# facebookresearch/PartDistillation

Hardware: AMD Instinct MI355X
Metric: images/sec training step, R50 Mask2Former 1024² bs=2/GPU, 1/2/4/8 MI355X (higher is better)
Workload: dtype bf16

## Files before the change

### partdistillation_amd/csrc/attention.hip

```cpp
#include <hip/hip_runtime.h>
#include <math.h>
#include <stdint.h>

#include "pd_attention.h"
#include "pd_common.h"
#include "mfma_bf16.h"
#include "pd_msda.h"

int g_attn_bwd_kc = 0;

namespace {

constexpr int D = 32;
constexpr int QP = 128;
constexpr int KT = 64;
constexpr int KC_FWD = 256;
constexpr int KC_DQ = 512;

typedef unsigned short bf16_t;

__device__ __forceinline__ float bf2f(bf16_t h) { return __uint_as_float((unsigned)h << 16); }
__device__ __forceinline__ bf16_t f2bf(float f)
{
  unsigned u = __float_as_uint(f);
  if ((u & 0x7fffffffu) > 0x7f800000u) return (bf16_t)((u >> 16) | 0x40);
  u += 0x7fffu + ((u >> 16) & 1u);
  return (bf16_t)(u >> 16);
}

template <typename T> struct IO;
template <> struct IO<float> {
  static __device__ __forceinline__ void load32(const float *p, float *dst)
  {
#pragma unroll
    for (int i = 0; i < 8; ++i) {
      const float4 v = reinterpret_cast<const float4 *>(p)[i];
      dst[4 * i] = v.x; dst[4 * i + 1] = v.y; dst[4 * i + 2] = v.z; dst[4 * i + 3] = v.w;
    }
  }
  static __device__ __forceinline__ void store32(float *p, const float *src)
  {
#pragma unroll
    for (int i = 0; i < 8; ++i) reinterpret_cast<float4 *>(p)[i] = make_float4(src[4 * i], src[4 * i + 1], src[4 * i + 2], src[4 * i + 3]);
  }
  static __device__ __forceinline__ void load8(const float *p, float *dst)
  {
    const float4 a = reinterpret_cast<const float4 *>(p)[0], b = reinterpret_cast<const float4 *>(p)[1];
    dst[0] = a.x; dst[1] = a.y; dst[2] = a.z; dst[3] = a.w; dst[4] = b.x; dst[5] = b.y; dst[6] = b.z; dst[7] = b.w;
  }
};
template <> struct IO<bf16_t> {
  static __device__ __forceinline__ void load8(const bf16_t *p, float *dst)
  {
    const uint4 v = *reinterpret_cast<const uint4 *>(p);
    const unsigned w[4] = {v.x, v.y, v.z, v.w};
#pragma unroll
    for (int i = 0; i < 4; ++i) { dst[2 * i] = __uint_as_float(w[i] << 16); dst[2 * i + 1] = __uint_as_float(w[i] & 0xffff0000u); }
  }
  static __device__ __forceinline__ void load32(const bf16_t *p, float *dst)
  {
#pragma unroll
    for (int i = 0; i < 4; ++i) load8(p + 8 * i, dst + 8 * i);
  }
  static __device__ __forceinline__ void store32(bf16_t *p, const float *src)
  {
#pragma unroll
    for (int i = 0; i < 4; ++i) {
      uint4 v;
      unsigned *w = &v.x;
#pragma unroll
      for (int j = 0; j < 4; ++j) w[j] = (unsigned)f2bf(src[8 * i + 2 * j]) | ((unsigned)f2bf(src[8 * i + 2 * j + 1]) << 16);
      reinterpret_cast<uint4 *>(p)[i] = v;
    }
  }
};

template <typename T>
__device__ __forceinline__ void stage_rows(const T *__restrict__ src, float (*dst)[D], int k0, int Lk, int b, int h, int B, int H)
{
  const int r = threadIdx.x >> 2, c = (threadIdx.x & 3) * 8;
  float tmp[8];
  if (k0 + r < Lk) IO<T>::load8(src + ((int64_t)(k0 + r) * B + b) * (H * D) + h * D + c, tmp);
  else {
#pragma unroll
    for (int i = 0; i < 8; ++i) tmp[i] = 0.f;
  }
#pragma unroll
  for (int i = 0; i < 8; ++i) dst[r][c + i] = tmp[i];
}

template <typename T>
__global__ __launch_bounds__(256) void attn_fwd_partial(const T *__restrict__ q, const T *__restrict__ k, const T *__restrict__ v,
// ... 200 lines not shown

template <typename T>
__global__ __launch_bounds__(256) void attn_bwd_dkv(const T *__restrict__ q, const T *__restrict__ k, const T *__restrict__ v,
                                                     const uint8_t *__restrict__ mask, const T *__restrict__ o, const T *__restrict__ d_o,
                                                     const float *__restrict__ lse, T *__restrict__ dk, T *__restrict__ dv, int B,
                                                     int H, int Lq, int Lk, float scale)
{
  __shared__ __attribute__((aligned(16))) float Qs[QS][D];
  __shared__ __attribute__((aligned(16))) float Os[QS][D];
  __shared__ float Ls[QS], Ds[QS];
  const int h = blockIdx.y, b = blockIdx.z;
  const int ki = blockIdx.x * 256 + threadIdx.x;
  const bool active = ki < Lk;
  float kv[D], vv[D], dkv[D], dvv[D];
#pragma unroll
  for (int d = 0; d < D; ++d) { dkv[d] = 0.f; dvv[d] = 0.f; }
  if (active) {
    const int64_t off = ((int64_t)ki * B + b) * (H * D) + h * D;
    IO<T>::load32(k + off, kv);
    IO<T>::load32(v + off, vv);
  }
  for (int q0 = 0; q0 < Lq; q0 += QS) {
    __syncthreads();
    {
      const int r = threadIdx.x >> 3, c = (threadIdx.x & 7) * 4;
      float part = 0.f;
      if (q0 + r < Lq) {
        const int64_t off = ((int64_t)(q0 + r) * B + b) * (H * D) + h * D + c;
#pragma unroll
        for (int i = 0; i < 4; ++i) {
          float qx, dox, ox;
          if (sizeof(T) == 2) {
            qx = bf2f(reinterpret_cast<const bf16_t *>(q)[off + i]); dox = bf2f(reinterpret_cast<const bf16_t *>(d_o)[off + i]);
            ox = bf2f(reinterpret_cast<const bf16_t *>(o)[off + i]);
          } else {
            qx = reinterpret_cast<const float *>(q)[off + i]; dox = reinterpret_cast<const float *>(d_o)[off + i];
            ox = reinterpret_cast<const float *>(o)[off + i];
          }
          Qs[r][c + i] = qx * scale; Os[r][c + i] = dox;
          part += dox * ox;
        }
      } else {
#pragma unroll
        for (int i = 0; i < 4; ++i) { Qs[r][c + i] = 0.f; Os[r][c + i] = 0.f; }
      }
      part += __shfl_xor(part, 1, 64); part += __shfl_xor(part, 2, 64); part += __shfl_xor(part, 4, 64);
      if ((threadIdx.x & 7) == 0) {
        Ds[r] = part;
        Ls[r] = (q0 + r < Lq) ? lse[((int64_t)b * H + h) * Lq + q0 + r] : -INFINITY;
      }
    }
    __syncthreads();
    if (!active) continue;
    const int nq = min(QS, Lq - q0);
    for (int r = 0; r < nq; ++r) {
      const float lq = Ls[r];
      if (lq == -INFINITY) continue;
      if (mask && mask[((int64_t)b * Lq + q0 + r) * Lk + ki]) continue;
      float s = 0.f, dp = 0.f;
#pragma unroll
      for (int d = 0; d < D; ++d) { s += Qs[r][d] * kv[d]; dp += Os[r][d] * vv[d]; }
      const float p = __expf(s - lq), ds = p * (dp - Ds[r]);
#pragma unroll
      for (int d = 0; d < D; ++d) { dkv[d] += ds * Qs[r][d]; dvv[d] += p * Os[r][d]; }
    }
  }
  if (active) {
    const int64_t off = ((int64_t)ki * B + b) * (H * D) + h * D;
    IO<T>::store32(dk + off, dkv);
    IO<T>::store32(dv + off, dvv);
  }
}

using pdmfma::bf16x4;
using pdmfma::f32x16;
using pdmfma::gather4;
using pdmfma::lds4;
using pdmfma::mma;
using pdmfma::pack4;

constexpr int LR = 36;
constexpr int LT = 132;
constexpr int MQ = 128;

__device__ __forceinline__ unsigned mask4(const uint8_t *row, int key0, int Lk, bool aligned)
{
  if (key0 >= Lk) return 0u;
  if (aligned) return *reinterpret_cast<const unsigned *>(row + key0);
  unsigned m = 0;
  for (int i = 0; i < 4; ++i)
    if (key0 + i < Lk) m |= (unsigned)row[key0 + i] << (8 * i);
  return m;
}

template <bool MASK>
__global__ __launch_bounds__(256) void attn_fwd_mfma(const bf16_t *__restrict__ q, const bf16_t *__restrict__ k,
                                                     const bf16_t *__restrict__ v, const uint8_t *__restrict__ mask,
                                                     bf16_t *__restrict__ o, float *__restrict__ lse, float *__restrict__ part_o,
                                                     float *__restrict__ part_ml, int B, int H, int Lq, int Lk, float scale,
                                                     int nchunk, int ldkv, int kc)
{
  __shared__ __attribute__((aligned(16))) bf16_t Ks[2][32][LR];
  __shared__ __attribute__((aligned(16))) bf16_t Vs[2][32][LR];
  const int chunk = blockIdx.x, h = blockIdx.y, b = blockIdx.z;
  const int tid = threadIdx.x, wave = tid >> 6, lane = tid & 63, r = lane & 31, hh = lane >> 5;
  const int qi = wave * 32 + r;
  const bool qvalid = qi < Lq;
  const int64_t rs = (int64_t)H * D;
  bf16x4 qreg[4];
#pragma unroll
  for (int s = 0; s < 4; ++s) {
    qreg[s] = bf16x4{0, 0, 0, 0};
    if (qvalid) qreg[s] = *reinterpret_cast<const bf16x4 *>(q + ((int64_t)qi * B + b) * rs + h * D + 8 * s + 4 * hh);
  }
  const int kbeg = chunk * kc, kend = min(Lk, kbeg + kc);
  const int ntile = (kend - kbeg + 31) / 32;
  const bf16_t *src = (tid < 128) ? k : v;
  const int srow = (tid & 127) >> 2, spiece = tid & 3;
  auto gload = [&](int t) {
    const int key = kbeg + 32 * t + srow;
    uint4 val = make_uint4(0, 0, 0, 0);
    if (key < kend) val = *reinterpret_cast<const uint4 *>(src + ((int64_t)key * B + b) * ldkv + h * D + spiece * 8);
    return val;
  };
  auto lstore = [&](int buf, uint4 val) {
    bf16_t *dst = ((tid < 128) ? &Ks[buf][srow][0] : &Vs[buf][srow][0]) + spiece * 8;
    *reinterpret_cast<uint2 *>(dst) = make_uint2(val.x, val.y);
    *reinterpret_cast<uint2 *>(dst + 4) = make_uint2(val.z, val.w);
  };
  const bool aligned = (Lk & 3) == 0;
  const uint8_t *mrow = (MASK && qvalid) ? mask + ((int64_t)b * Lq + qi) * Lk : nullptr;
  float m_run = -INFINITY, l_part = 0.f;
  f32x16 oacc;
#pragma unroll
  for (int e = 0; e < 16; ++e) oacc[e] = 0.f;
  if (ntile > 0) lstore(0, gload(0));
  __syncthreads();
  for (int t = 0; t < ntile; ++t) {
    const int buf = t & 1, kbase = kbeg + 32 * t;
    uint4 nxt = make_uint4(0, 0, 0, 0);
    if (t + 1 < ntile) nxt = gload(t + 1);
    f32x16 sacc;
#pragma unroll
    for (int e = 0; e < 16; ++e) sacc[e] = 0.f;
#pragma unroll
    for (int s = 0; s < 4; ++s) mma(sacc, lds4(&Ks[buf][r][8 * s + 4 * hh]), qreg[s]);
    float m_t = -INFINITY;
#pragma unroll
    for (int g = 0; g < 4; ++g) {
      const int key0 = kbase + 8 * g + 4 * hh;
      const unsigned m4 = mrow ? mask4(mrow, key0, Lk, aligned) : 0u;
#pragma unroll
      for (int i = 0; i < 4; ++i) {
        const bool blocked = (key0 + i >= kend) || ((m4 >> (8 * i)) & 0xffu);
        const float sv = blocked ? -INFINITY : sacc[4 * g + i] * scale;
        sacc[4 * g + i] = sv;
        m_t = fmaxf(m_t, sv);
      }
    }
    m_t = fmaxf(m_t, __shfl_xor(m_t, 32, 64));
    const float m_new = fmaxf(m_run, m_t);
    const bool dead = m_new == -INFINITY;
    const float alpha = dead ? 1.f : __expf(m_run - m_new);
    float psum = 0.f;
    bf16x4 preg[4];
#pragma unroll
// ... 149 lines not shown
#pragma unroll
          for (int s = 0; s < 4; ++s) { mma(sT, kreg[s], qreg[s]); mma(dpT, vreg[s], greg[s]); }
          const float lse_q = Ls[ql], delta_q = Ds[ql];
          unsigned mybits = 0;
          bf16x4 dsT[4];
#pragma unroll
          for (int g = 0; g < 4; ++g) {
            const int key0 = kbase + 8 * g + 4 * hh;
            const unsigned m4 = m4s[sub][g];
            float ds[4];
#pragma unroll
            for (int i = 0; i < 4; ++i) {
              const bool blocked = (key0 + i >= kend) || ((m4 >> (8 * i)) & 0xffu);
              const float p = blocked ? 0.f : __expf(sT[4 * g + i] * scale - lse_q);
              ds[i] = p * (dpT[4 * g + i] - delta_q);
              const unsigned long long bal = __ballot(blocked);
              if (r == 8 * g + i) mybits = (unsigned)bal;
              if (r == 8 * g + 4 + i) mybits = (unsigned)(bal >> 32);
            }
            dsT[g] = pack4(ds[0], ds[1], ds[2], ds[3]);
          }
#pragma unroll
          for (int j = 0; j < 4; ++j) mma(dqacc[sub], ktreg[j], dsT[j]);
          f32x16 sN, dpN;
#pragma unroll
          for (int e = 0; e < 16; ++e) { sN[e] = 0.f; dpN[e] = 0.f; }
#pragma unroll
          for (int s = 0; s < 4; ++s) { mma(sN, qreg[s], kreg[s]); mma(dpN, greg[s], vreg[s]); }
          bf16x4 pN[4], dsN[4];
#pragma unroll
          for (int g = 0; g < 4; ++g) {
            const float4 l4 = *reinterpret_cast<const float4 *>(&Ls[32 * sub + 8 * g + 4 * hh]);
            const float4 d4 = *reinterpret_cast<const float4 *>(&Ds[32 * sub + 8 * g + 4 * hh]);
            const float la[4] = {l4.x, l4.y, l4.z, l4.w}, da[4] = {d4.x, d4.y, d4.z, d4.w};
            float p[4], ds[4];
#pragma unroll
            for (int i = 0; i < 4; ++i) {
              const bool blocked = (mybits >> (8 * g + 4 * hh + i)) & 1u;
              p[i] = blocked ? 0.f : __expf(sN[4 * g + i] * scale - la[i]);
              ds[i] = p[i] * (dpN[4 * g + i] - da[i]);
            }
            pN[g] = pack4(p[0], p[1], p[2], p[3]);
            dsN[g] = pack4(ds[0], ds[1], ds[2], ds[3]);
          }
#pragma unroll
          for (int j = 0; j < 4; ++j) {
            mma(dvacc, lds4(&Ot[r][32 * sub + 8 * j + 4 * hh]), pN[j]);
            mma(dkacc, lds4(&Qt[r][32 * sub + 8 * j + 4 * hh]), dsN[j]);
          }
        }
      }
      if (kvalid) {
        bf16_t *dkp = dk + ((int64_t)key * B + b) * rs + h * D, *dvp = dv + ((int64_t)key * B + b) * rs + h * D;
#pragma unroll
        for (int g = 0; g < 4; ++g) {
          *reinterpret_cast<bf16x4 *>(dkp + 8 * g + 4 * hh) = pack4(dkacc[4 * g] * scale, dkacc[4 * g + 1] * scale, dkacc[4 * g + 2] * scale, dkacc[4 * g + 3] * scale);
          *reinterpret_cast<bf16x4 *>(dvp + 8 * g + 4 * hh) = pack4(dvacc[4 * g], dvacc[4 * g + 1], dvacc[4 * g + 2], dvacc[4 * g + 3]);
        }
      }
    }
  }
  for (int w = 0; w < 4; ++w) {
    __syncthreads();
    if (wave == w) {
#pragma unroll
      for (int sub = 0; sub < 4; ++sub)
#pragma unroll
        for (int e = 0; e < 16; ++e) {
          const int d = (e & 3) + 8 * (e >> 2) + 4 * hh;
          if (w == 0) dqs[32 * sub + r][d] = dqacc[sub][e];
          else dqs[32 * sub + r][d] += dqacc[sub][e];
        }
    }
  }
  __syncthreads();
  for (int idx = tid; idx < Lq * D; idx += 256) {
    const int qq = idx >> 5, d = idx & 31;
    const float val = dqs[qq][d] * scale;
    if (nchunk == 1) dq[((int64_t)qq * B + b) * rs + h * D + d] = f2bf(val);
    else part_dq[((bh * nchunk + chunk) * Lq + qq) * D + d] = val;
  }
}

inline int nchunks(int Lk, int kc) { return Lk <= 0 ? 1 : (Lk + kc - 1) / kc; }
inline int mfma_fwd_chunk(int B, int H, int Lk)
{
  int kc = KC_FWD;
  if (Lk > KC_FWD)
    while (kc > 64 && (int64_t)B * H * nchunks(Lk, kc) < 512) kc >>= 1;
  return kc;
}
inline int mfma_bwd_chunk(int B, int H, int Lk)
{
  if (g_attn_bwd_kc == 128 || g_attn_bwd_kc == 256 || g_attn_bwd_kc == 512) return g_attn_bwd_kc;
  int kc = KC_DQ;
  while (kc > 128 && (int64_t)B * H * nchunks(Lk, kc) < 256) kc >>= 1;
  return kc;
}

int check(const void *a, const void *b, const void *c, int B, int H, int Lq, int Lk, int dtype, const char *who)
{
  if (B < 0 || H <= 0 || Lq < 0 || Lk < 0) return pd_set_error(PD_ERR_INVALID_ARG, "%s: bad sizes B=%d H=%d Lq=%d Lk=%d", who, B, H, Lq, Lk);
  if (dtype != PD_F32 && dtype != PD_BF16) return pd_set_error(PD_ERR_INVALID_ARG, "%s: dtype %d (float32 / bfloat16 only)", who, dtype);
  if (B * Lq * Lk != 0 && (!a || !b || !c)) return pd_set_error(PD_ERR_INVALID_ARG, "%s: null pointer", who);
  return PD_OK;
}

}

int g_pd_dbg_attn_scalar = 0;

extern "C" int64_t pd_attn_workspace_floats(int B, int H, int Lq, int Lk)
{
  const int64_t n1 = (int64_t)B * H * nchunks(Lk, mfma_fwd_chunk(B, H, Lk)) * Lq * (D + 2);
  const int64_t n2 = (int64_t)B * H * nchunks(Lk, 128) * Lq * D;
  return (n1 > n2 ? n1 : n2) + 64;
}

extern "C" int pd_attn_fwd_d32(const void *q, const void *k, const void *v, const uint8_t *mask, void *o, float *lse,
                               float *workspace, int B, int H, int Lq, int Lk, float scale, int dtype, void *stream_)
{
  return pd_attn_fwd_d32_ld(q, k, v, mask, o, lse, workspace, B, H, Lq, Lk, scale, dtype, H * D, stream_);
}

extern "C" int pd_attn_fwd_d32_ld(const void *q, const void *k, const void *v, const uint8_t *mask, void *o, float *lse,
                                  float *workspace, int B, int H, int Lq, int Lk, float scale, int dtype, int ld_kv, void *stream_)
{
  int rc = check(q, k, v, B, H, Lq, Lk, dtype, "pd_attn_fwd_d32");
  if (rc) return rc;
  if (ld_kv < H * D || (ld_kv & 7)) return pd_set_error(PD_ERR_INVALID_ARG, "pd_attn_fwd_d32_ld: ld_kv=%d (>= H * 32, a multiple of 8)", ld_kv);
  if (ld_kv != H * D && !(dtype == PD_BF16 && Lq <= MQ && Lk > 0 && !g_pd_dbg_attn_scalar))
    return pd_set_error(PD_ERR_INVALID_ARG, "pd_attn_fwd_d32_ld: strided k / v only on the matrix-core path (bf16, <= %d queries)", MQ);
  if (B * Lq == 0) return PD_OK;
  if (!o || !lse || !workspace) return pd_set_error(PD_ERR_INVALID_ARG, "pd_attn_fwd_d32: null output");
  hipStream_t s = (hipStream_t)stream_;
  if (dtype == PD_BF16 && Lq <= MQ && Lk > 0 && !g_pd_dbg_attn_scalar) {
    const int kc = mfma_fwd_chunk(B, H, Lk), nc = nchunks(Lk, kc);
    float *part_o = workspace, *part_ml = workspace + (int64_t)B * H * nc * Lq * D;
    if (mask) hipLaunchKernelGGL(attn_fwd_mfma<true>, dim3(nc, H, B), dim3(256), 0, s, (const bf16_t *)q, (const bf16_t *)k, (const bf16_t *)v,
                                 mask, (bf16_t *)o, lse, part_o, part_ml, B, H, Lq, Lk, scale, nc, ld_kv, kc);
    else hipLaunchKernelGGL(attn_fwd_mfma<false>, dim3(nc, H, B), dim3(256), 0, s, (const bf16_t *)q, (const bf16_t *)k, (const bf16_t *)v,
                            mask, (bf16_t *)o, lse, part_o, part_ml, B, H, Lq, Lk, scale, nc, ld_kv, kc);
    if (nc > 1) hipLaunchKernelGGL(attn_fwd_combine<bf16_t>, dim3((B * H * Lq + 7) / 8), dim3(256), 0, s, part_o, part_ml, (bf16_t *)o, lse, B, H, Lq, nc);
    return pd_check_launch("pd_attn_fwd_d32");
  }
  const int nc = nchunks(Lk, KC_FWD);
  float *part_o = workspace, *part_ml = workspace + (int64_t)B * H * nc * Lq * D;
  for (int qp = 0; qp * QP < Lq; ++qp) {
    if (dtype == PD_BF16)
      hipLaunchKernelGGL(attn_fwd_partial<bf16_t>, dim3(nc, H, B), dim3(256), 0, s, (const bf16_t *)q, (const bf16_t *)k,
                         (const bf16_t *)v, mask, part_o, part_ml, B, H, Lq, Lk, scale, nc, qp);
    else
      hipLaunchKernelGGL(attn_fwd_partial<float>, dim3(nc, H, B), dim3(256), 0, s, (const float *)q, (const float *)k,
                         (const float *)v, mask, part_o, part_ml, B, H, Lq, Lk, scale, nc, qp);
  }
  const int groups = B * H * Lq;
  if (dtype == PD_BF16)
    hipLaunchKernelGGL(attn_fwd_combine<bf16_t>, dim3((groups + 7) / 8), dim3(256), 0, s, part_o, part_ml, (bf16_t *)o, lse, B, H, Lq, nc);
  else
    hipLaunchKernelGGL(attn_fwd_combine<float>, dim3((groups + 7) / 8), dim3(256), 0, s, part_o, part_ml, (float *)o, lse, B, H, Lq, nc);
  return pd_check_launch("pd_attn_fwd_d32");
}

extern "C" int pd_attn_bwd_d32(const void *q, const void *k, const void *v, const uint8_t *mask, const void *o, const void *d_o,
                               const float *lse, void *dq, void *dk, void *dv, float *workspace, int B, int H, int Lq,
                               int Lk, float scale, int dtype, void *stream_)
{
  return pd_attn_bwd_d32_ld(q, k, v, mask, o, d_o, lse, dq, dk, dv, workspace, B, H, Lq, Lk, scale, dtype, H * D, stream_);
}

extern "C" int pd_attn_bwd_d32_ld(const void *q, const void *k, const void *v, const uint8_t *mask, const void *o, const void *d_o,
                                  const float *lse, void *dq, void *dk, void *dv, float *workspace, int B, int H, int Lq,
                                  int Lk, float scale, int dtype, int ld_kv, void *stream_)
{
  int rc = check(q, k, v, B, H, Lq, Lk, dtype, "pd_attn_bwd_d32");
  if (rc) return rc;
  if (ld_kv < H * D || (ld_kv & 3)) return pd_set_error(PD_ERR_INVALID_ARG, "pd_attn_bwd_d32_ld: ld_kv=%d (>= H * 32, a multiple of 4)", ld_kv);
  if (ld_kv != H * D && !(dtype == PD_BF16 && Lq <= MQ && !g_pd_dbg_attn_scalar))
    return pd_set_error(PD_ERR_INVALID_ARG, "pd_attn_bwd_d32_ld: strided k / v only on the matrix-core path (bf16, <= %d queries)", MQ);
  hipStream_t s = (hipStream_t)stream_;
  if (B * Lq == 0) {
    const size_t bytes = (size_t)B * Lk * H * D * (dtype == PD_BF16 ? 2 : 4);
    if (bytes == 0) return PD_OK;
    if (!dk || !dv) return pd_set_error(PD_ERR_INVALID_ARG, "pd_attn_bwd_d32: null pointer");
    if (hipMemsetAsync(dk, 0, bytes, s) != hipSuccess || hipMemsetAsync(dv, 0, bytes, s) != hipSuccess)
      return pd_set_error(PD_ERR_LAUNCH, "pd_attn_bwd_d32: clearing dk / dv failed");
    return PD_OK;
  }
  const int groups = B * H * Lq;
  if (Lk == 0) {
    if (!dq) return pd_set_error(PD_ERR_INVALID_ARG, "pd_attn_bwd_d32: null pointer");
    if (dtype == PD_BF16) hipLaunchKernelGGL(attn_bwd_dq_reduce<bf16_t>, dim3((groups + 7) / 8), dim3(256), 0, s, workspace, (bf16_t *)dq, B, H, Lq, 0);
    else hipLaunchKernelGGL(attn_bwd_dq_reduce<float>, dim3((groups + 7) / 8), dim3(256), 0, s, workspace, (float *)dq, B, H, Lq, 0);
    return pd_check_launch("pd_attn_bwd_d32");
  }
  if (!o || !d_o || !lse || !dq || !dk || !dv || !workspace) return pd_set_error(PD_ERR_INVALID_ARG, "pd_attn_bwd_d32: null pointer");
  if (dtype == PD_BF16 && Lq <= MQ && !g_pd_dbg_attn_scalar) {
    const int kc = mfma_bwd_chunk(B, H, Lk), nc = nchunks(Lk, kc);
    if (mask) hipLaunchKernelGGL(attn_bwd_mfma<true>, dim3(nc, H, B), dim3(256), 0, s, (const bf16_t *)q, (const bf16_t *)k, (const bf16_t *)v,
                                 mask, (const bf16_t *)o, (const bf16_t *)d_o, lse, workspace, (bf16_t *)dq, (bf16_t *)dk, (bf16_t *)dv,
                                 B, H, Lq, Lk, scale, nc, kc, ld_kv);
    else hipLaunchKernelGGL(attn_bwd_mfma<false>, dim3(nc, H, B), dim3(256), 0, s, (const bf16_t *)q, (const bf16_t *)k, (const bf16_t *)v,
                            mask, (const bf16_t *)o, (const bf16_t *)d_o, lse, workspace, (bf16_t *)dq, (bf16_t *)dk, (bf16_t *)dv,
                            B, H, Lq, Lk, scale, nc, kc, ld_kv);
    if (nc > 1) hipLaunchKernelGGL(attn_bwd_dq_reduce<bf16_t>, dim3((groups + 7) / 8), dim3(256), 0, s, workspace, (bf16_t *)dq, B, H, Lq, nc);
    return pd_check_launch("pd_attn_bwd_d32");
  }
  const int nc = nchunks(Lk, KC_DQ);
  if (dtype == PD_BF16) {
    for (int qp = 0; qp * QP < Lq; ++qp)
      hipLaunchKernelGGL(attn_bwd_dq<bf16_t>, dim3(nc, H, B), dim3(256), 0, s, (const bf16_t *)q, (const bf16_t *)k, (const bf16_t *)v,
                         mask, (const bf16_t *)o, (const bf16_t *)d_o, lse, workspace, B, H, Lq, Lk, scale, nc, qp);
    hipLaunchKernelGGL(attn_bwd_dq_reduce<bf16_t>, dim3((groups + 7) / 8), dim3(256), 0, s, workspace, (bf16_t *)dq, B, H, Lq, nc);
    hipLaunchKernelGGL(attn_bwd_dkv<bf16_t>, dim3((Lk + 255) / 256, H, B), dim3(256), 0, s, (const bf16_t *)q, (const bf16_t *)k,
                       (const bf16_t *)v, mask, (const bf16_t *)o, (const bf16_t *)d_o, lse, (bf16_t *)dk, (bf16_t *)dv, B, H, Lq, Lk, scale);
  } else {
    for (int qp = 0; qp * QP < Lq; ++qp)
      hipLaunchKernelGGL(attn_bwd_dq<float>, dim3(nc, H, B), dim3(256), 0, s, (const float *)q, (const float *)k, (const float *)v,
                         mask, (const float *)o, (const float *)d_o, lse, workspace, B, H, Lq, Lk, scale, nc, qp);
    hipLaunchKernelGGL(attn_bwd_dq_reduce<float>, dim3((groups + 7) / 8), dim3(256), 0, s, workspace, (float *)dq, B, H, Lq, nc);
    hipLaunchKernelGGL(attn_bwd_dkv<float>, dim3((Lk + 255) / 256, H, B), dim3(256), 0, s, (const float *)q, (const float *)k,
                       (const float *)v, mask, (const float *)o, (const float *)d_o, lse, (float *)dk, (float *)dv, B, H, Lq, Lk, scale);
  }
  return pd_check_launch("pd_attn_bwd_d32");
}
```

### partdistillation_amd/csrc/common.hip

```cpp
#include <hip/hip_runtime.h>
#include <stdarg.h>
#include <stdio.h>
#include <string.h>

#include "pd_common.h"
#include "pd_msda.h"

namespace {
thread_local char g_err[512] = {0};
}

int pd_set_error(int code, const char *fmt, ...)
{
  va_list ap;
  va_start(ap, fmt);
  vsnprintf(g_err, sizeof(g_err), fmt, ap);
  va_end(ap);
  return code;
}

int pd_check_launch(const char *what)
{
  hipError_t e = hipGetLastError();
  if (e == hipSuccess) return PD_OK;
  return pd_set_error(PD_ERR_LAUNCH, "%s: %s", what, hipGetErrorString(e));
}

extern "C" const char *pd_last_error(void) { return g_err; }
extern "C" int pd_abi_version(void) { return PD_ABI_VERSION; }

extern int g_pd_dbg_atomic_scope;
extern int g_pd_dbg_force_generic;
extern int g_pd_dbg_ablate;
extern int g_pd_dbg_f16x2;
extern int g_pd_dbg_wgrad_wide;
extern "C" void pd_dbg_set_wgrad_xcd(int v);
extern "C" void pd_dbg_set_wgrad_fast(int v);
extern int g_pd_dbg_bwd_variant;
extern int g_pd_dbg_msda_gate_pct;
extern int g_pd_dbg_wgrad_wgs;
extern int g_pd_dbg_bwd_threads;
extern int g_pd_dbg_attn_scalar;
extern int g_pd_dbg_wattn;
extern int g_pd_dbg_wattn_chunk;
extern int g_pd_dbg_kmeans;
extern int g_pd_dbg_conv_group_rows;
extern int g_pd_dbg_conv_xcd_major;
extern int g_pd_dbg_sgemm_deep;
extern int g_ig_bn, g_ig_nst, g_ig_splits, g_ig_patch, g_ig_pcls;
extern int g_mx_bn, g_mx_nst;
extern int g_swin_ln_abl;
extern int g_ln_bwd_cap;
extern int g_crit_abl;
extern int g_attn_bwd_kc;
extern int g_wg_nst, g_wg_splits, g_wg_mode;
extern "C" int pd_debug_set(const char *key, int value)
{
  if (!key) return PD_ERR_INVALID_ARG;
  if (!strcmp(key, "msda_bwd_atomic_scope")) { g_pd_dbg_atomic_scope = value; return PD_OK; }
  if (!strcmp(key, "msda_ablate")) { g_pd_dbg_ablate = value; return PD_OK; }
  if (!strcmp(key, "msda_bwd_variant")) { g_pd_dbg_bwd_variant = value; return PD_OK; }
  if (!strcmp(key, "msda_gate_pct")) { g_pd_dbg_msda_gate_pct = value; return PD_OK; }
  if (!strcmp(key, "attn_scalar")) { g_pd_dbg_attn_scalar = value; return PD_OK; }
  if (!strcmp(key, "msda_bwd_threads")) { g_pd_dbg_bwd_threads = value; return PD_OK; }
  if (!strcmp(key, "wgrad_wgs")) { g_pd_dbg_wgrad_wgs = value; return PD_OK; }
  if (!strcmp(key, "kmeans_ablate")) { g_pd_dbg_kmeans = value; return PD_OK; }
  if (!strcmp(key, "wg_nst")) { g_wg_nst = value; return PD_OK; }
  if (!strcmp(key, "wg_splits")) { g_wg_splits = value; return PD_OK; }
  if (!strcmp(key, "wg_mode")) { g_wg_mode = value; return PD_OK; }
  if (!strcmp(key, "ig_bn")) { g_ig_bn = value; return PD_OK; }
  if (!strcmp(key, "ig_patch")) { g_ig_patch = value; return PD_OK; }
  if (!strcmp(key, "ig_pcls")) { g_ig_pcls = value; return PD_OK; }
  if (!strcmp(key, "ig_nst")) { g_ig_nst = value; return PD_OK; }
  if (!strcmp(key, "mx_bn")) { g_mx_bn = value; return PD_OK; }
  if (!strcmp(key, "attn_bwd_kc")) { g_attn_bwd_kc = value; return PD_OK; }
  if (!strcmp(key, "crit_abl")) { g_crit_abl = value; return PD_OK; }
  if (!strcmp(key, "ln_bwd_cap")) { g_ln_bwd_cap = value; return PD_OK; }
  if (!strcmp(key, "swin_ln_abl")) { g_swin_ln_abl = value; return PD_OK; }
  if (!strcmp(key, "mx_nst")) { g_mx_nst = value; return PD_OK; }
  if (!strcmp(key, "ig_splits")) { g_ig_splits = value; return PD_OK; }
  if (!strcmp(key, "sgemm_deep")) { g_pd_dbg_sgemm_deep = value; return PD_OK; }
  if (!strcmp(key, "conv_group_rows")) { g_pd_dbg_conv_group_rows = value; return PD_OK; }
  if (!strcmp(key, "conv_xcd_major")) { g_pd_dbg_conv_xcd_major = value; return PD_OK; }
  if (!strcmp(key, "f16x2_tile")) { g_pd_dbg_f16x2 = value; return PD_OK; }
  if (!strcmp(key, "wgrad_wide")) { g_pd_dbg_wgrad_wide = value; return PD_OK; }
  if (!strcmp(key, "wgrad_xcd")) { pd_dbg_set_wgrad_xcd(value); return PD_OK; }
  if (!strcmp(key, "wgrad_fast")) { pd_dbg_set_wgrad_fast(value); return PD_OK; }
  if (!strcmp(key, "wattn_ablate")) { g_pd_dbg_wattn = value; return PD_OK; }
  if (!strcmp(key, "wattn_chunk")) {
    if (value < 0 || value > 8) return pd_set_error(PD_ERR_INVALID_ARG, "pd_debug_set: wattn_chunk is 0 (automatic) or 1..8, got %d", value);
    g_pd_dbg_wattn_chunk = value;
    return PD_OK;
  }
  if (!strcmp(key, "msda_force_generic")) { g_pd_dbg_force_generic = value; return PD_OK; }
  return pd_set_error(PD_ERR_INVALID_ARG, "pd_debug_set: unknown key %s", key);
}

extern "C" int pd_debug_get(const char *key, int *value)
{
  if (!key || !value) return PD_ERR_INVALID_ARG;
  if (!strcmp(key, "msda_bwd_variant")) { *value = g_pd_dbg_bwd_variant; return PD_OK; }
  if (!strcmp(key, "msda_gate_pct")) { *value = g_pd_dbg_msda_gate_pct; return PD_OK; }
  return pd_set_error(PD_ERR_INVALID_ARG, "pd_debug_get: unknown key %s", key);
}
```

### partdistillation_amd/csrc/mfma_bf16.h

```cpp
#ifndef PD_MFMA_BF16_H
#define PD_MFMA_BF16_H
#include <hip/hip_runtime.h>

namespace pdmfma {

typedef unsigned short bf16_t;
typedef short bf16x4 __attribute__((ext_vector_type(4)));
typedef float f32x16 __attribute__((ext_vector_type(16)));
typedef __bf16 hwbf16x2 __attribute__((ext_vector_type(2)));
typedef float f32x2 __attribute__((ext_vector_type(2)));

__device__ __forceinline__ unsigned pk_bf16(float lo, float hi)
{
  const f32x2 x = {lo, hi};
  return __builtin_bit_cast(unsigned, __builtin_convertvector(x, hwbf16x2));
}
__device__ __forceinline__ bf16x4 pack4(float a, float b, float c, float d)
{
  union { unsigned u[2]; bf16x4 v; } x;
  x.u[0] = pk_bf16(a, b); x.u[1] = pk_bf16(c, d);
  return x.v;
}
__device__ __forceinline__ float bf_lo(unsigned u) { return __uint_as_float(u << 16); }
__device__ __forceinline__ float bf_hi(unsigned u) { return __uint_as_float(u & 0xffff0000u); }
__device__ __forceinline__ void mma(f32x16 &c, bf16x4 x, bf16x4 y) { c = __builtin_amdgcn_mfma_f32_32x32x8bf16_1k(x, y, c, 0, 0, 0); }
__device__ __forceinline__ bf16x4 lds4(const bf16_t *p) { return *reinterpret_cast<const bf16x4 *>(p); }
__device__ __forceinline__ bf16x4 gather4(const bf16_t *p, int stride)
{
  bf16x4 r;
  r[0] = (short)p[0]; r[1] = (short)p[stride]; r[2] = (short)p[2 * stride]; r[3] = (short)p[3 * stride];
  return r;
}

}
#endif
```

Baseline: 110.2.

## Add transposed-LDS attention backward kernel with deeper MFMA and key-tile prefetch

Adds a new attention backward kernel used by default (form 3). It uses ds_read_tr16 transposed LDS reads instead of scalar gathers for K^T, Q^T and dO^T operands, and computes dS once per tile, staging it through LDS for the dQ product rather than recomputing a transposed S. It uses the 32x32x16 bf16 MFMA, prefetches the next key tile and mask into registers, and sets launch bounds for two blocks per SM. This adds LDS use and register pressure and relies on gfx950-specific instructions. Older forms stay selectable through a debug key.

```diff
diff --git a/partdistillation_amd/csrc/attention.hip b/partdistillation_amd/csrc/attention.hip
--- a/partdistillation_amd/csrc/attention.hip
+++ b/partdistillation_amd/csrc/attention.hip
@@ -8,6 +8,7 @@
 #include "pd_msda.h"
 
 int g_attn_bwd_kc = 0;
+int g_attn_bwd_form = 3;
 
 namespace {
 
@@ -374,6 +375,7 @@
 constexpr int LR = 36;
 constexpr int LT = 132;
 constexpr int MQ = 128;
+constexpr int LM = 36;
 
 __device__ __forceinline__ unsigned mask4(const uint8_t *row, int key0, int Lk, bool aligned)
 {
@@ -689,6 +691,235 @@
   }
 }
 
+template <bool MASK, int FORM>
+__global__ __launch_bounds__(256, 2) void attn_bwd_mfma_tr(const bf16_t *__restrict__ q, const bf16_t *__restrict__ k,
+                                                        const bf16_t *__restrict__ v, const uint8_t *__restrict__ mask,
+                                                        const bf16_t *__restrict__ o, const bf16_t *__restrict__ d_o,
+                                                        const float *__restrict__ lse, float *__restrict__ part_dq,
+                                                        bf16_t *__restrict__ dq, bf16_t *__restrict__ dk, bf16_t *__restrict__ dv,
+                                                        int B, int H, int Lq, int Lk, float scale, int nchunk, int kc, int ldkv)
+{
+  constexpr bool ONCE = FORM >= 2, DEEP = FORM >= 3;
+  __shared__ __attribute__((aligned(16))) bf16_t QO[2][MQ][LR];
+  __shared__ __attribute__((aligned(16))) float Ls[MQ];
+  __shared__ __attribute__((aligned(16))) float Ds[MQ];
+  __shared__ __attribute__((aligned(16))) bf16_t Kw[4][32][LR];
+  __shared__ __attribute__((aligned(16))) bf16_t Sw[ONCE ? 4 : 1][32][LR];
+  __shared__ __attribute__((aligned(16))) uint8_t Mw[(ONCE && MASK) ? 4 : 1][MQ][LM];
+  static_assert(sizeof(QO) >= sizeof(float) * 4 * 32 * (D + 1), "dqs aliases the Q / dO tiles");
+  bf16_t (*Qs)[LR] = QO[0], (*Os)[LR] = QO[1];
+  float (*dqs)[32][D + 1] = reinterpret_cast<float (*)[32][D + 1]>(&QO[0][0][0]);
+  const int chunk = blockIdx.x, h = blockIdx.y, b = blockIdx.z;
+  const int tid = threadIdx.x, wave = tid >> 6, lane = tid & 63, r = lane & 31, hh = lane >> 5;
+  const int64_t rs = (int64_t)H * D;
+  const int64_t bh = (int64_t)b * H + h;
+  const int kbeg = chunk * kc, kend = min(Lk, kbeg + kc);
+  const int ntile = (kend - kbeg + 31) / 32;
+  const int nsub = (Lq + 31) / 32;
+  const bool aligned = (Lk & 3) == 0;
+  constexpr bool AHEAD = ONCE;
+  bf16x4 kn[4], vn[4];
+  unsigned mn[4][4];
+  auto load_tile = [&](int t) {
+    const int kbase = kbeg + 32 * t, key = min(kbase + r, kend - 1);
+#pragma unroll
+    for (int s = 0; s < 4; ++s) {
+      const int64_t off = ((int64_t)key * B + b) * ldkv + h * D + 8 * s + 4 * hh;
+      kn[s] = *reinterpret_cast<const bf16x4 *>(k + off);
+      vn[s] = *reinterpret_cast<const bf16x4 *>(v + off);
+    }
+#pragma unroll
+    for (int sub = 0; sub < 4; ++sub) {
+      const int ql = 32 * sub + r;
+      const uint8_t *mrow = (MASK && sub < nsub && ql < Lq) ? mask + ((int64_t)b * Lq + ql) * Lk : nullptr;
+#pragma unroll
+      for (int g = 0; g < 4; ++g) mn[sub][g] = mrow ? mask4(mrow, kbase + 8 * g + 4 * hh, Lk, aligned) : 0u;
+    }
+  };
+  if (AHEAD && wave < ntile) load_tile(wave);
+  constexpr int NP = MQ * 4 / 256;
+  uint4 qv[NP], gv[NP], ov[NP];
+  float lv[NP];
+#pragma unroll
+  for (int it = 0; it < NP; ++it) {
+    const int row = (tid + 256 * it) >> 2, piece = tid & 3;
+    const int64_t off = ((int64_t)(row < Lq ? row : 0) * B + b) * rs + h * D + piece * 8;
+    qv[it] = *reinterpret_cast<const uint4 *>(q + off);
+    gv[it] = *reinterpret_cast<const uint4 *>(d_o + off);
+    ov[it] = *reinterpret_cast<const uint4 *>(o + off);
+    lv[it] = lse[bh * Lq + (row < Lq ? row : 0)];
+  }
+#pragma unroll
+  for (int it = 0; it < NP; ++it) {
+    const int row = (tid + 256 * it) >> 2, piece = tid & 3;
+    if (row >= Lq) { qv[it] = make_uint4(0, 0, 0, 0); gv[it] = qv[it]; ov[it] = qv[it]; }
+    *reinterpret_cast<uint2 *>(&Qs[row][piece * 8]) = make_uint2(qv[it].x, qv[it].y);
+    *reinterpret_cast<uint2 *>(&Qs[row][piece * 8 + 4]) = make_uint2(qv[it].z, qv[it].w);
+    *reinterpret_cast<uint2 *>(&Os[row][piece * 8]) = make_uint2(gv[it].x, gv[it].y);
+    *reinterpret_cast<uint2 *>(&Os[row][piece * 8 + 4]) = make_uint2(gv[it].z, gv[it].w);
+    const unsigned ga[4] = {gv[it].x, gv[it].y, gv[it].z, gv[it].w}, oa[4] = {ov[it].x, ov[it].y, ov[it].z, ov[it].w};
+    float part = 0.f;
+#pragma unroll
+    for (int i = 0; i < 4; ++i)
+      part += bf2f((bf16_t)(ga[i] & 0xffffu)) * bf2f((bf16_t)(oa[i] & 0xffffu)) + bf2f((bf16_t)(ga[i] >> 16)) * bf2f((bf16_t)(oa[i] >> 16));
+    part += __shfl_xor(part, 1, 64);
+    part += __shfl_xor(part, 2, 64);
+    if (piece == 0) {
+      Ds[row] = part;
+      Ls[row] = (row >= Lq || lv[it] == -INFINITY) ? INFINITY : lv[it];
+    }
+  }
+  __syncthreads();
+  const int troff = pdmfma::tr_offset(lane, LR);
+  const bf16_t *kt_tile = &Kw[wave][0][0] + troff, *st_tile = &Sw[ONCE ? wave : 0][0][0] + troff;
+  const bf16_t *qt_tile = &Qs[0][0] + troff, *ot_tile = &Os[0][0] + troff;
+  f32x16 dqacc[4];
+#pragma unroll
+  for (int s = 0; s < 4; ++s)
+#pragma unroll
+    for (int e = 0; e < 16; ++e) dqacc[s][e] = 0.f;
+  for (int t = wave; t < ntile; t += 4) {
+    const int kbase = kbeg + 32 * t;
+    const int key = kbase + r;
+    const bool kvalid = key < kend;
+    if (!AHEAD) load_tile(t);
+    bf16x4 kreg[4], vreg[4];
+    unsigned m4s[4][4];
+#pragma unroll
+    for (int s = 0; s < 4; ++s) { kreg[s] = kvalid ? kn[s] : bf16x4{0, 0, 0, 0}; vreg[s] = kvalid ? vn[s] : bf16x4{0, 0, 0, 0}; }
+#pragma unroll
+    for (int sub = 0; sub < 4; ++sub)
+#pragma unroll
+      for (int g = 0; g < 4; ++g) m4s[sub][g] = mn[sub][g];
+    pdmfma::wave_lds_order();
+#pragma unroll
+    for (int s = 0; s < 4; ++s) *reinterpret_cast<bf16x4 *>(&Kw[wave][r][8 * s + 4 * hh]) = kreg[s];
+    if constexpr (ONCE && MASK) {
+#pragma unroll
+      for (int sub = 0; sub < 4; ++sub)
+        if (sub < nsub) {
+#pragma unroll
+          for (int g = 0; g < 4; ++g) *reinterpret_cast<unsigned *>(&Mw[wave][32 * sub + r][8 * g + 4 * hh]) = m4s[sub][g];
+        }
+    }
+    pdmfma::wave_lds_order();
+    if (AHEAD && t + 4 < ntile) load_tile(t + 4);
+    bf16x4 ktreg[4];
+#pragma unroll
+    for (int j = 0; j < 4; ++j) ktreg[j] = pdmfma::lds4_tr(kt_tile + 8 * j * LR);
+    f32x16 dkacc, dvacc;
+#pragma unroll
+    for (int e = 0; e < 16; ++e) { dkacc[e] = 0.f; dvacc[e] = 0.f; }
+#pragma unroll
+    for (int sub = 0; sub < 4; ++sub) {
+      if (sub < nsub) {
+        const int ql = 32 * sub + r;
+        bf16x4 qreg[4], greg[4];
+#pragma unroll
+        for (int s = 0; s < 4; ++s) {
+          qreg[s] = lds4(&Qs[ql][8 * s + 4 * hh]);
+          greg[s] = lds4(&Os[ql][8 * s + 4 * hh]);
+        }
+        unsigned mybits = 0;
+        bf16x4 dsT[4];
+        if constexpr (!ONCE) {
+          f32x16 sT, dpT;
+#pragma unroll
+          for (int e = 0; e < 16; ++e) { sT[e] = 0.f; dpT[e] = 0.f; }
+#pragma unroll
+          for (int s = 0; s < 4; ++s) { mma(sT, kreg[s], qreg[s]); mma(dpT, vreg[s], greg[s]); }
+          const float lse_q = Ls[ql], delta_q = Ds[ql];
+#pragma unroll
+          for (int g = 0; g < 4; ++g) {
+            const int key0 = kbase + 8 * g + 4 * hh;
+            const unsigned m4 = m4s[sub][g];
+            float ds[4];
+#pragma unroll
+            for (int i = 0; i < 4; ++i) {
+              const bool blocked = (key0 + i >= kend) || ((m4 >> (8 * i)) & 0xffu);
+              const float p = blocked ? 0.f : __expf(sT[4 * g + i] * scale - lse_q);
+              ds[i] = p * (dpT[4 * g + i] - delta_q);
+              const unsigned long long bal = __ballot(blocked);
+              if (r == 8 * g + i) mybits = (unsigned)bal;
+              if (r == 8 * g + 4 + i) mybits = (unsigned)(bal >> 32);
+            }
+            dsT[g] = pack4(ds[0], ds[1], ds[2], ds[3]);
+          }
+#pragma unroll
+          for (int j = 0; j < 4; ++j) mma(dqacc[sub], ktreg[j], dsT[j]);
+        }
+        f32x16 sN, dpN;
+#pragma unroll
+        for (int e = 0; e < 16; ++e) { sN[e] = 0.f; dpN[e] = 0.f; }
+        pdmfma::mma32<DEEP>(sN, qreg, kreg);
+        pdmfma::mma32<DEEP>(dpN, greg, vreg);
+        bf16x4 pN[4], dsN[4];
+#pragma unroll
+        for (int g = 0; g < 4; ++g) {
+          const float4 l4 = *reinterpret_cast<const float4 *>(&Ls[32 * sub + 8 * g + 4 * hh]);
+          const float4 d4 = *reinterpret_cast<const float4 *>(&Ds[32 * sub + 8 * g + 4 * hh]);
+          const float la[4] = {l4.x, l4.y, l4.z, l4.w}, da[4] = {d4.x, d4.y, d4.z, d4.w};
+          float p[4], ds[4];
+#pragma unroll
+          for (int i = 0; i < 4; ++i) {
+            unsigned blocked;
+            if constexpr (ONCE) blocked = (MASK ? (unsigned)Mw[wave][32 * sub + 8 * g + 4 * hh + i][r] : 0u) | (unsigned)!kvalid;
+            else blocked = (mybits >> (8 * g + 4 * hh + i)) & 1u;
+            const float pe = __expf(sN[4 * g + i] * scale - la[i]);
+            p[i] = blocked ? 0.f : pe;
+            ds[i] = p[i] * (dpN[4 * g + i] - da[i]);
+          }
+          pN[g] = pack4(p[0], p[1], p[2], p[3]);
+          dsN[g] = pack4(ds[0], ds[1], ds[2], ds[3]);
+        }
+        bf16x4 otreg[4], qtreg[4];
+#pragma unroll
+        for (int j = 0; j < 4; ++j) {
+          otreg[j] = pdmfma::lds4_tr(ot_tile + (32 * sub + 8 * j) * LR);
+          qtreg[j] = pdmfma::lds4_tr(qt_tile + (32 * sub + 8 * j) * LR);
+        }
+        pdmfma::mma32<DEEP>(dvacc, otreg, pN);
+        pdmfma::mma32<DEEP>(dkacc, qtreg, dsN);
+        if constexpr (ONCE) {
+          pdmfma::wave_lds_order();
+#pragma unroll
+          for (int g = 0; g < 4; ++g) *reinterpret_cast<bf16x4 *>(&Sw[wave][r][8 * g + 4 * hh]) = dsN[g];
+          pdmfma::wave_lds_order();
+#pragma unroll
+          for (int j = 0; j < 4; ++j) dsT[j] = pdmfma::lds4_tr(st_tile + 8 * j * LR);
+          pdmfma::mma32<DEEP>(dqacc[sub], ktreg, dsT);
+        }
+      }
+    }
+    if (kvalid) {
+      bf16_t *dkp = dk + ((int64_t)key * B + b) * rs + h * D, *dvp = dv + ((int64_t)key * B + b) * rs + h * D;
+#pragma unroll
+      for (int g = 0; g < 4; ++g) {
+        *reinterpret_cast<bf16x4 *>(dkp + 8 * g + 4 * hh) = pack4(dkacc[4 * g] * scale, dkacc[4 * g + 1] * scale, dkacc[4 * g + 2] * scale, dkacc[4 * g + 3] * scale);
+        *reinterpret_cast<bf16x4 *>(dvp + 8 * g + 4 * hh) = pack4(dvacc[4 * g], dvacc[4 * g + 1], dvacc[4 * g + 2], dvacc[4 * g + 3]);
+      }
+    }
+  }
+#pragma unroll
+  for (int sub = 0; sub < 4; ++sub) {
+    if (sub < nsub) {
+      __syncthreads();
+#pragma unroll
+      for (int e = 0; e < 16; ++e) dqs[wave][r][(e & 3) + 8 * (e >> 2) + 4 * hh] = dqacc[sub][e];
+      __syncthreads();
+#pragma unroll
+      for (int j = 0; j < 4; ++j) {
+        const int idx = tid + 256 * j, ql = idx >> 5, d = idx & 31, qq = 32 * sub + ql;
+        const float val = (((dqs[0][ql][d] + dqs[1][ql][d]) + dqs[2][ql][d]) + dqs[3][ql][d]) * scale;
+        if (qq < Lq) {
+          if (nchunk == 1) dq[((int64_t)qq * B + b) * rs + h * D + d] = f2bf(val);
+          else part_dq[((bh * nchunk + chunk) * Lq + qq) * D + d] = val;
+        }
+      }
+    }
+  }
+}
+
 inline int nchunks(int Lk, int kc) { return Lk <= 0 ? 1 : (Lk + kc - 1) / kc; }
 inline int mfma_fwd_chunk(int B, int H, int Lk)
 {
@@ -804,12 +1035,16 @@
   if (!o || !d_o || !lse || !dq || !dk || !dv || !workspace) return pd_set_error(PD_ERR_INVALID_ARG, "pd_attn_bwd_d32: null pointer");
   if (dtype == PD_BF16 && Lq <= MQ && !g_pd_dbg_attn_scalar) {
     const int kc = mfma_bwd_chunk(B, H, Lk), nc = nchunks(Lk, kc);
-    if (mask) hipLaunchKernelGGL(attn_bwd_mfma<true>, dim3(nc, H, B), dim3(256), 0, s, (const bf16_t *)q, (const bf16_t *)k, (const bf16_t *)v,
-                                 mask, (const bf16_t *)o, (const bf16_t *)d_o, lse, workspace, (bf16_t *)dq, (bf16_t *)dk, (bf16_t *)dv,
-                                 B, H, Lq, Lk, scale, nc, kc, ld_kv);
-    else hipLaunchKernelGGL(attn_bwd_mfma<false>, dim3(nc, H, B), dim3(256), 0, s, (const bf16_t *)q, (const bf16_t *)k, (const bf16_t *)v,
-                            mask, (const bf16_t *)o, (const bf16_t *)d_o, lse, workspace, (bf16_t *)dq, (bf16_t *)dk, (bf16_t *)dv,
-                            B, H, Lq, Lk, scale, nc, kc, ld_kv);
+#define PD_ATTN_BWD_LAUNCH(KERNEL)                                                                                                          \
+  hipLaunchKernelGGL(KERNEL, dim3(nc, H, B), dim3(256), 0, s, (const bf16_t *)q, (const bf16_t *)k, (const bf16_t *)v, mask, (const bf16_t *)o, \
+                     (const bf16_t *)d_o, lse, workspace, (bf16_t *)dq, (bf16_t *)dk, (bf16_t *)dv, B, H, Lq, Lk, scale, nc, kc, ld_kv)
+    switch (g_attn_bwd_form) {
+    case 0: if (mask) PD_ATTN_BWD_LAUNCH(attn_bwd_mfma<true>); else PD_ATTN_BWD_LAUNCH(attn_bwd_mfma<false>); break;
+    case 1: if (mask) PD_ATTN_BWD_LAUNCH((attn_bwd_mfma_tr<true, 1>)); else PD_ATTN_BWD_LAUNCH((attn_bwd_mfma_tr<false, 1>)); break;
+    case 2: if (mask) PD_ATTN_BWD_LAUNCH((attn_bwd_mfma_tr<true, 2>)); else PD_ATTN_BWD_LAUNCH((attn_bwd_mfma_tr<false, 2>)); break;
+    default: if (mask) PD_ATTN_BWD_LAUNCH((attn_bwd_mfma_tr<true, 3>)); else PD_ATTN_BWD_LAUNCH((attn_bwd_mfma_tr<false, 3>)); break;
+    }
+#undef PD_ATTN_BWD_LAUNCH
     if (nc > 1) hipLaunchKernelGGL(attn_bwd_dq_reduce<bf16_t>, dim3((groups + 7) / 8), dim3(256), 0, s, workspace, (bf16_t *)dq, B, H, Lq, nc);
     return pd_check_launch("pd_attn_bwd_d32");
   }
diff --git a/partdistillation_amd/csrc/common.hip b/partdistillation_amd/csrc/common.hip
--- a/partdistillation_amd/csrc/common.hip
+++ b/partdistillation_amd/csrc/common.hip
@@ -52,7 +52,7 @@
 extern int g_swin_ln_abl;
 extern int g_ln_bwd_cap;
 extern int g_crit_abl;
-extern int g_attn_bwd_kc;
+extern int g_attn_bwd_kc, g_attn_bwd_form;
 extern int g_wg_nst, g_wg_splits, g_wg_mode;
 extern "C" int pd_debug_set(const char *key, int value)
 {
@@ -74,6 +74,11 @@
   if (!strcmp(key, "ig_nst")) { g_ig_nst = value; return PD_OK; }
   if (!strcmp(key, "mx_bn")) { g_mx_bn = value; return PD_OK; }
   if (!strcmp(key, "attn_bwd_kc")) { g_attn_bwd_kc = value; return PD_OK; }
+  if (!strcmp(key, "attn_bwd_form")) {
+    if (value < 0 || value > 3) return pd_set_error(PD_ERR_INVALID_ARG, "pd_debug_set: attn_bwd_form is 0 .. 3, got %d", value);
+    g_attn_bwd_form = value;
+    return PD_OK;
+  }
   if (!strcmp(key, "crit_abl")) { g_crit_abl = value; return PD_OK; }
   if (!strcmp(key, "ln_bwd_cap")) { g_ln_bwd_cap = value; return PD_OK; }
   if (!strcmp(key, "swin_ln_abl")) { g_swin_ln_abl = value; return PD_OK; }
@@ -101,5 +106,6 @@
   if (!key || !value) return PD_ERR_INVALID_ARG;
   if (!strcmp(key, "msda_bwd_variant")) { *value = g_pd_dbg_bwd_variant; return PD_OK; }
   if (!strcmp(key, "msda_gate_pct")) { *value = g_pd_dbg_msda_gate_pct; return PD_OK; }
+  if (!strcmp(key, "attn_bwd_form")) { *value = g_attn_bwd_form; return PD_OK; }
   return pd_set_error(PD_ERR_INVALID_ARG, "pd_debug_get: unknown key %s", key);
 }
diff --git a/partdistillation_amd/csrc/mfma_bf16.h b/partdistillation_amd/csrc/mfma_bf16.h
--- a/partdistillation_amd/csrc/mfma_bf16.h
+++ b/partdistillation_amd/csrc/mfma_bf16.h
@@ -32,5 +32,41 @@
   return r;
 }
 
+__device__ __forceinline__ int tr_offset(int lane, int pitch)
+{
+  const int c = lane & 15;
+  return (4 * (lane >> 5) + (c >> 2)) * pitch + 16 * ((lane >> 4) & 1) + 4 * (c & 3);
+}
+__device__ __forceinline__ bf16x4 lds4_tr(const bf16_t *p)
+{
+  typedef __attribute__((address_space(3))) bf16x4 *lp;
+  return __builtin_amdgcn_ds_read_tr16_b64_v4i16((lp)p);
+}
+__device__ __forceinline__ void wave_lds_order()
+{
+  asm volatile("" ::: "memory");
+  __builtin_amdgcn_wave_barrier();
+  asm volatile("" ::: "memory");
+}
+
+typedef short bf16x8 __attribute__((ext_vector_type(8)));
+typedef __bf16 hwbf16x8 __attribute__((ext_vector_type(8)));
+__device__ __forceinline__ void mma16(f32x16 &c, bf16x4 x0, bf16x4 x1, bf16x4 y0, bf16x4 y1)
+{
+  const bf16x8 x = __builtin_shufflevector(x0, x1, 0, 1, 2, 3, 4, 5, 6, 7), y = __builtin_shufflevector(y0, y1, 0, 1, 2, 3, 4, 5, 6, 7);
+  c = __builtin_amdgcn_mfma_f32_32x32x16_bf16(__builtin_bit_cast(hwbf16x8, x), __builtin_bit_cast(hwbf16x8, y), c, 0, 0, 0);
+}
+template <bool DEEP>
+__device__ __forceinline__ void mma32(f32x16 &c, const bf16x4 (&x)[4], const bf16x4 (&y)[4])
+{
+  if constexpr (DEEP) {
+    mma16(c, x[0], x[1], y[0], y[1]);
+    mma16(c, x[2], x[3], y[2], y[3]);
+  } else {
+#pragma unroll
+    for (int s = 0; s < 4; ++s) mma(c, x[s], y[s]);
+  }
+}
+
 }
 #endif
```

New measurement: 111.2, median of 6. No clear change (+0.9%).
